# navigator8972/vae_assoc

Hardware: AMD Instinct MI355X
Metric: paired-samples/sec (img+jnt assoc-VAE train step) (higher is better)
Workload: dtype bf16

## Files before the change

vae_assoc_amd/csrc/avae_device.h:

```cpp
#pragma once
#include <hip/hip_runtime.h>
#include <stdint.h>

namespace avae {

constexpr int kMaxMod = 4;
constexpr int kThreads = 256;
constexpr int kTileBytesK = 128;
constexpr int kRowAlign = 256;
constexpr int kLatentRows = 16;
constexpr int kAdamRows = 16;
constexpr int kCostHist = 4096;

enum Kind : int {
    K_FWD_HIDDEN = 0,
    K_FWD_HEAD = 1,
    K_FWD_OUT_LOSS = 2,
    K_FWD_OUT_STORE = 3,
    K_DGRAD_HIDDEN = 4,
    K_DGRAD_LATENT = 5,
    K_WGRAD = 6,
    K_DGRAD_F32 = 10,
    K_LATENT = 7,
    K_COST = 8,
// ... 54 lines not shown
    int src_sb, src_sp;
    int ones;
    unsigned mg_ohw, mg_ow, mg_k, mg_cin;
};
constexpr int kMaxConvA = 12;
constexpr int kMaxItemsPerLaunch = 12;
constexpr int kMaxPf = 4;
struct LaunchArgs {
    int n_items;
    int grid_x;
    int sched;
    int n_pf;
    const void* pf_ptr[4];
    int pf_lines[4];
    const ConvA* conv_tab;
    WorkItem items[kMaxItemsPerLaunch];
};

struct TnItem {
    const void* A;
    const void* B;
    float* out;
    int M, N, K;
    int lda, ldb, ld0;
    int tiles_m, tiles_n;
    int ksplit, kchunk;
    int bias_row;
    int tile_off, tile_cnt;
    int conv;
    void* W; void* Wt;
    int ldw, ldt;
};
constexpr int kMaxTnItems = 32;
constexpr int kTnPieces = 8;
struct TnPiece { unsigned short item, tile_off, cum_end, pad; };
struct DevState;
struct TnLaunchArgs {
    int n_items;
    int grid_x;
    int xcd_group;
    int sched;
    int adam;
    long long d_theta, d_m, d_v;
    float beta1, beta2, eps;
    const DevState* st;
    const ConvA* conv_tab;
    int xcd_pieces;
    TnPiece pieces[8][kTnPieces];
    TnItem items[kMaxTnItems];
};
static_assert(sizeof(TnLaunchArgs) <= 4096, "kernel arguments are passed by value: 4 KiB");

struct DevState {
    long long step;
    float last_cost;
    float lr_t;
    float cost_hist[kCostHist];
};

struct AdamItem {
    float* theta;
    float* m;
    float* v;
    const float* g;
    void* W;
    void* Wt;
    int rows, cols;
    int ld, ldt;
    int tiles_r, tiles_c, tile_base;
    int ldw;
    void* Wadj; void* Wf;
    int ldadj, ldf, adj_k, adj_cin;
};

constexpr int kMaxAdamItems = 80;
struct AdamArgs {
    const AdamItem* items;
    int n_items;
    int base[kMaxAdamItems];
    int mode;
    int book;
// ... 219 lines not shown
```

vae_assoc_amd/csrc/avae_host.hip:

```cpp
#include "avae_device.h"
#include "../../include/avae.h"

#include <dlfcn.h>
#include <sched.h>
#include <unistd.h>

#include <algorithm>
#include <cmath>
#include <cstdio>
#include <cstdlib>
#include <cstring>
#include <functional>
#include <map>
#include <mutex>
#include <stdexcept>
#include <string>
#include <vector>

using namespace avae;

namespace {

thread_local std::string g_create_error;

// ... 168 lines not shown
    int bwd_split = 0;
    std::vector<Launch> wgrad_b[2];
    struct Range { size_t off, count; };
    std::vector<Range> ranges_b[2];
    int adam_first_b[2] = {0, 0}, adam_count_b[2] = {0, 0}, adam_blocks_b[2] = {0, 0};
    std::vector<AdamItem> adam_items_b;
    size_t off_adam_b = 0;
    void* comm = nullptr;
    int comm_world = 1, comm_rank = 0;
    bool comm_on = false;
    size_t off_wire = 0;
    unsigned char* ipc_block = nullptr;
    size_t ipc_bytes = 0;
    unsigned char* ipc_peer[kMaxWorld] = {nullptr, nullptr, nullptr, nullptr, nullptr, nullptr, nullptr, nullptr};
    bool ipc_opened[kMaxWorld] = {false, false, false, false, false, false, false, false};
    bool ipc_attached = false;
    IpcArgs ipc_args{};
    hipStream_t comm_stream = nullptr;
    hipEvent_t ev_grad[2] = {nullptr, nullptr}, ev_red[2] = {nullptr, nullptr};
    std::vector<StepGraph> g_dp[2];
    StepGraph g_dpm[2];
    bool dp_graph_failed = false;
    Launch cost_only;
    std::vector<AdamItem> adam_items;
    int adam_blocks = 0;
    struct Inf { std::vector<WorkItem> items; std::vector<Launch> launches; int rows = -1; size_t dev_off = 0; };
    std::vector<Inf> inf_enc, inf_dec;
    struct Serve { int bucket = 0; std::vector<WorkItem> items; std::vector<Launch> launches; hipGraphExec_t graph = nullptr; ServeArgs in;
                   Launch in_launch; bool fused_in = false;
                   ServeInArgs in_lean; int in_lean_grid = 0; bool lean_in = false; };
    std::vector<Serve> serve;
    size_t off_slot = 0;
    float* iw_buf = nullptr;
    size_t off_chain = 0;
    size_t off_consts = 0, off_conv_tab = 0;
    std::vector<ConvA> conv_tab;

    StepPlan plain, masked;
    unsigned char* pres_buf = nullptr;
    size_t pres_set = 0;

    hipStream_t last_stream = nullptr;
    bool has_last_stream = false;
    hipEvent_t ev_switch = nullptr;
    unsigned draw_id = 0;
    bool timing = false;
    bool debug_sync = false;
    std::vector<std::string> tnames;
    std::vector<TimingRec> trecs;

    template <typename T> T* at(size_t off) const { return reinterpret_cast<T*>(ws + off); }
    DevState* state() const { return at<DevState>(off_state); }
    float* grad() const { return at<float>(off_g); }
};

namespace {

inline int spread_ld(int ld, int KU, int es) {
    static const bool off = std::getenv("AVAE_NO_LD_SPREAD") != nullptr;
    return (!off && ((size_t)ld * es) % 512 == 0) ? ld + KU : ld;
}

Act make_act(Bump& b, int width, bool ones, int rows, int KU, int es, int ld = 0) {
    Act a;
    a.width = width;
    a.rows = rows;
// ... 751 lines not shown
            std::vector<std::vector<TnItem>> bins, bins2;
            if (!std::getenv("AVAE_TN_G") && G == 4 && n * 2 <= kMaxTnItems * 2) {
                const long r4 = pack(4, bins), r2 = pack(2, bins2);
                if (r2 < r4) { G = 2; bins.swap(bins2); }
            } else {
                pack(G, bins);
            }
            size_t groups = 0;
            for (const auto& bn : bins) groups = std::max(groups, bn.size());
            std::memset(L.targs.items, 0, sizeof(L.targs.items));
            for (size_t g = 0; g < groups; ++g)
                for (int p = 0; p < G; ++p) if (g < bins[p].size()) L.targs.items[g * G + p] = bins[p][g];
            n = (int)groups * G;
        }
        L.grid_x = SX;
        L.targs.n_items = n;
        L.targs.grid_x = L.grid_x;
        L.targs.xcd_group = G;
        L.grid_y = (n + G - 1) / G * G;
        L.blocks = L.grid_x * L.grid_y;
    } else {
        L.args.n_items = count;
        L.args.grid_x = L.grid_x;
        for (int i = 0; i < count; ++i) L.args.items[i] = items[first + i];
    }
    L.args.conv_tab = L.targs.conv_tab = h->at<ConvA>(h->off_conv_tab);
    if (const char* e = std::getenv("AVAE_SCHED")) L.args.sched = L.targs.sched = std::atoi(e);
    if (*next_slot > h->n_partial) throw Err("internal error: cost partial slots overflow");
    return L;
}

void dp_ranges(const avae_handle* h, int* n_buckets, std::vector<avae_handle::Range> (&out)[2]);

void xcd_pieces(Launch& L) {
    TnLaunchArgs& a = L.targs;
    std::vector<TnItem> layers;
    for (int i = 0; i < a.n_items; ++i) {
        const TnItem& e = a.items[i];
        if (e.tile_cnt <= 0) continue;
        bool seen = false;
        for (const TnItem& l : layers) seen = seen || l.out == e.out;
        if (seen) continue;
        TnItem l = e;
        l.tile_off = 0; l.tile_cnt = e.tiles_m * e.tiles_n;
        if (l.tile_cnt > 65535) return;
        layers.push_back(l);
    }
    long total = 0;
    for (const TnItem& l : layers) total += l.tile_cnt;
    if (layers.empty() || total > 8L * 65535) return;
    const int quota = (int)((total + 7) / 8);
    std::vector<int> order(layers.size());
    for (size_t i = 0; i < order.size(); ++i) order[i] = (int)i;
    std::stable_sort(order.begin(), order.end(), [&](int x, int y) { return layers[x].tile_cnt > layers[y].tile_cnt; });
    struct Bin { int load = 0; std::vector<TnPiece> pc; };
    Bin bins[8];
    for (int li : order) {
        int off = 0, left = layers[li].tile_cnt;
        while (left > 0) {
            int best = -1;
            for (int b = 0; b < 8; ++b)
                if ((int)bins[b].pc.size() < kTnPieces && bins[b].load + left <= quota && (best < 0 || bins[b].load > bins[best].load)) best = b;
            int take = left;
            if (best < 0) {
                for (int b = 0; b < 8; ++b)
                    if ((int)bins[b].pc.size() < kTnPieces && bins[b].load < quota && (best < 0 || bins[b].load < bins[best].load)) best = b;
                if (best < 0) return;
                take = std::min(left, quota - bins[best].load);
            }
            bins[best].load += take;
            bins[best].pc.push_back(TnPiece{(unsigned short)li, (unsigned short)off, (unsigned short)bins[best].load, 0});
            off += take; left -= take;
        }
    }
    int longest = 0;
    for (int b = 0; b < 8; ++b) {
        longest = std::max(longest, bins[b].load);
        for (int i = 0; i < kTnPieces; ++i)
            a.pieces[b][i] = i < (int)bins[b].pc.size() ? bins[b].pc[i] : TnPiece{0, 0, (unsigned short)bins[b].load, 0};
    }
    std::memset(a.items, 0, sizeof(a.items));
    for (size_t i = 0; i < layers.size(); ++i) a.items[i] = layers[i];
    a.n_items = (int)layers.size();
    a.xcd_pieces = 1;
    L.grid_x = 8 * longest; L.grid_y = 1; L.blocks = L.grid_x;
    a.grid_x = L.grid_x;
}

void build_training_plan(avae_handle* h) {
    h->items.clear(); h->plain.fwd.clear(); h->bwd.clear(); h->wgrad.clear(); h->conv_tab.clear();
    Builder bd(h, h->items, h->B, true);
    int slot = 0;
    int Lmax = 0;
    for (const Mod& md : h->mods) Lmax = std::max(Lmax, md.L);
    auto group = [&](const std::string& name, std::vector<Launch>& dst, auto&& fill) {
        const int first = (int)h->items.size();
        fill();
        const int count = (int)h->items.size() - first;
        if (count <= 0) return;
        dst.push_back(finish_launch(h, h->items, first, count, name, &slot));
    };
    auto fuse_tail = [&](std::vector<Launch>& ls, int mode) {
        if (ls.size() < 2 || std::getenv("AVAE_NO_TAIL")) return false;
        Launch& Lp = ls[ls.size() - 2];
        Launch& Lc = ls[ls.size() - 1];
        if (Lp.type != 0 || Lc.type != 0 || Lp.tn || Lc.tn || Lp.cfg != 3) return false;
        const int want_p = mode == 1 ? K_FWD_HEAD : K_DGRAD_LATENT, want_c = mode == 1 ? K_FWD_HIDDEN : K_DGRAD_HIDDEN;
        std::vector<int> prod(Lc.count, -1);
        for (int i = 0; i < Lc.count; ++i) {
            const WorkItem& c = h->items[Lc.first + i];
            if (c.kind != want_c || c.bias_ep || c.K > 2 * h->KU || c.N > 1024) return false;
            for (int k = 0; k < Lp.count; ++k) {
                const WorkItem& n = h->items[Lp.first + k];
                if (n.kind != want_p || n.M != c.M) continue;
                const void* res = mode == 1 ? n.out1 : n.out0;
                const int ldres = mode == 1 ? n.ld1 : n.ld0;
                if (res && res == c.A && ldres == c.lda) prod[i] = k;
            }
// ... 495 lines not shown
                g.block_base = base; base += (st.g.Cin * st.g.k * st.g.k * st.d.out + kThreads - 1) / kThreads;
            }
            L.blocks = base;
            if (base > 0) h->wgrad.push_back(L);
        }
    }
    h->wgrad_adam.clear();
    if (!any_conv && h->wgrad.size() == 1 && h->wgrad[0].tn && h->wgrad[0].cfg == 0 && h->wgrad[0].targs.xcd_group == 1
        && !std::getenv("AVAE_NO_LEAN") && !std::getenv("AVAE_NO_ADAM_FUSE")) {
        Launch L = h->wgrad[0];
        bool ok = true;
        for (int i = 0; i < L.targs.n_items && ok; ++i) {
            TnItem& t = L.targs.items[i];
            ok = t.ksplit <= 1 && t.bias_row == 0 && t.K > 0;
            const Dense* dm = nullptr;
            for (const Mod& md : h->mods) {
                auto look = [&](const Dense& d) { if (h->grad() + d.master == t.out) dm = &d; };
                for (const Dense& d : md.enc) look(d);
                look(md.head);
                for (const Dense& d : md.dec) look(d);
                look(md.outl);
            }
            ok = ok && dm && t.M == dm->in + 1 && t.N == dm->out && t.ld0 == dm->ld;
            if (ok) { t.W = h->at<void>(dm->W); t.Wt = h->at<void>(dm->Wt); t.ldw = dm->ldw; t.ldt = dm->ldt; }
        }
        if (ok) {
            L.cfg = 12; L.name = "wgrad+adam";
            L.targs.adam = 1;
            L.targs.d_theta = h->at<float>(h->off_theta) - h->grad();
            L.targs.d_m = h->at<float>(h->off_m) - h->grad();
            L.targs.d_v = h->at<float>(h->off_v) - h->grad();
            L.targs.beta1 = h->cfg.beta1; L.targs.beta2 = h->cfg.beta2; L.targs.eps = h->cfg.adam_eps;
            L.targs.st = h->state();
            if (!std::getenv("AVAE_NO_XCD_PIECES")) xcd_pieces(L);
            h->wgrad_adam.push_back(L);
        }
    }
    if (!std::getenv("AVAE_NO_WARM")) {
        std::vector<Launch*> seq;
        for (Launch& L : h->plain.fwd) seq.push_back(&L);
        for (Launch& L : h->bwd) seq.push_back(&L);
        for (size_t i = 0; i < seq.size(); ++i) {
            Launch& L = *seq[i];
            if (L.type != 0 || L.tn || (L.cfg != 2 && L.cfg != 6)) continue;
            for (size_t j = i + 1; j < seq.size(); ++j) {
                const Launch& Nx = *seq[j];
                if (Nx.type != 0) continue;
                if (Nx.tn) break;
                for (int k = 0; k < Nx.args.n_items && L.args.n_pf < kMaxPf; ++k) {
                    const WorkItem& w = Nx.args.items[k];
                    if (!is_gemm(w.kind) || w.kind == K_WGRAD) continue;
                    const long bytes = (long)w.N * w.ldb * h->es;
                    if (bytes < 128 * 1024) continue;
                    L.args.pf_ptr[L.args.n_pf] = w.B; L.args.pf_lines[L.args.n_pf] = (int)(bytes / 128); ++L.args.n_pf;
                }
                break;
            }
        }
    }
    {
        const int first = (int)h->items.size();
        h->items.push_back(bd.cost(false));
        h->cost_only = finish_launch(h, h->items, first, 1, "cost_reduce", &slot);
    }

    h->adam_items.clear();
    int base = 0;
// ... 116 lines not shown
    avae_handle* h; hipStream_t s; bool on; hipEvent_t a = nullptr, b = nullptr; int id = 0;
    Timed(avae_handle* h_, hipStream_t s_, const std::string& name) : h(h_), s(s_), on(h_->timing && h_->trecs.size() < 200000) {
        if (!on) return;
        id = tname_id(h, name);
        HIP_OK(hipEventCreate(&a)); HIP_OK(hipEventCreate(&b));
        t_launch_events = LaunchEvents{a, b};
    }
    ~Timed() {
        if (!on) return;
        if (t_launch_events.start) {
            t_launch_events = LaunchEvents{nullptr, nullptr};
            (void)hipEventRecord(a, s); (void)hipEventRecord(b, s);
        }
        h->trecs.push_back(TimingRec{a, b, id});
    }
};

Launch relocated(const avae_handle* h, const Launch& L0, int j) {
    Launch L = L0;
    const unsigned char* lo = h->ws + h->stage_lo;
    const unsigned char* hi = lo + h->stage_bytes;
    const size_t delta = (size_t)j * h->stage_bytes;
    auto fix = [&](auto& ptr) {
        const unsigned char* q = reinterpret_cast<const unsigned char*>(ptr);
        if (q >= lo && q < hi) ptr = reinterpret_cast<std::remove_reference_t<decltype(ptr)>>(const_cast<unsigned char*>(q) + delta);
    };
    for (int i = 0; i < L.args.n_items && L.type == 0; ++i) {
        WorkItem& w = L.args.items[i];
        fix(w.A); fix(w.B); fix(w.out0); fix(w.out1); fix(w.out2); fix(w.aux0); fix(w.aux1); fix(w.aux2); fix(w.eps);
        fix(w.tail_w); fix(w.tail_out); fix(w.tail_aux);
        if (w.present) w.present += (size_t)j * h->pres_set;
    }
    for (int i = 0; i < L.targs.n_items && L.type == 0; ++i) { TnItem& t = L.targs.items[i]; fix(t.A); fix(t.B); fix(t.out); }
    for (int i = 0; i < L.ga.n_seg && L.type == 1; ++i) fix(L.ga.seg[i].src);
    return L;
}

void run_launch(avae_handle* h, const Launch& L, hipStream_t s, unsigned long long* stamps, int stamp) {
    Timed t(h, s, L.name);
    if (L.type == 1) launch_gather(h->cfg.compute_dtype, L.ga, L.blocks, s);
    else if (L.type == 2) launch_col2im(h->cfg.compute_dtype, L.ca, L.blocks, s);
    else if (L.type == 3) launch_reduce(L.ra, L.blocks, s);
    else if (L.type == 4) launch_thin(h->cfg.compute_dtype, L.ta, L.blocks, s);
    else if (L.type == 5) launch_colsum(L.ra, L.blocks, s);
    else if (L.type == 6) launch_wadj(h->cfg.compute_dtype, L.wa, L.blocks, s);
    else if (L.type == 7) launch_gperm(L.gp, L.blocks, s);
    else if (L.type == 8) launch_rowsum(h->cfg.compute_dtype, L.rs, L.blocks, s);
    else if (L.type == 9) launch_sums(L.ra, L.blocks, s);
    else if (L.cfg == 13) launch_chain2(h->cfg.compute_dtype, L.args, L.grid_x, L.grid_y, L.lds, h->at<unsigned>(h->off_chain), h->at<unsigned>(h->off_chain) + kMaxMod * 64, s);
    else if (L.cfg == 11) launch_small_head(h->cfg.compute_dtype, L.lean_act, L.args, L.grid_x, L.grid_y, L.lds, s, stamps, stamp);
    else if (L.cfg == 10) launch_small_latb(h->cfg.compute_dtype, L.lean_act, L.args, L.grid_x, L.grid_y, L.lds, h->state(), s, stamps, stamp);
    else if (L.cfg == 9) launch_small_loss(h->cfg.compute_dtype, L.args, L.grid_x, L.grid_y, L.lds, s, stamps, stamp);
    else if (L.cfg == 7) launch_small(h->cfg.compute_dtype, L.args, L.grid_x, L.grid_y, L.lds, s, stamps, stamp);
    else if (L.tn && L.cfg == 12) launch_small_tn(h->cfg.compute_dtype, L.targs, L.grid_x, L.grid_y, s, stamps, stamp);
    else if (L.tn) launch_grouped_tn(h->cfg.compute_dtype, L.cfg, L.targs, L.grid_x, L.grid_y, L.lds, h->state(), s, stamps, stamp);
    else launch_grouped(h->cfg.compute_dtype, L.cfg, L.args, L.grid_x, L.grid_y, L.lds, h->state(), s, stamps, stamp);
    LAUNCH_OK(L.name);
    if (h->debug_sync) {
        std::fprintf(stderr, "[avae] launch %s type=%d cfg=%d items=%d blocks=%d\n", L.name.c_str(), L.type, L.cfg, L.count, L.blocks);
        for (int i = 0; i < L.args.n_items && L.type == 0; ++i)
            std::fprintf(stderr, "        item kind=%d M=%d N=%d K=%d lda=%d ldb=%d tiles=%dx%d\n", L.args.items[i].kind, L.args.items[i].M,
                         L.args.items[i].N, L.args.items[i].K, L.args.items[i].lda, L.args.items[i].ldb, L.args.items[i].tiles_m, L.args.items[i].tiles_n);
        for (int i = 0; i < L.ga.n_seg && L.type == 1; ++i)
            std::fprintf(stderr, "        gather B=%d IH=%d Cin=%d OH=%d k=%d so=%d d=%d pad=%d sb=%d sp=%d ones=%d ldp=%d tiles=%dx%d\n", L.ga.seg[i].g.B, L.ga.seg[i].g.IH,
                         L.ga.seg[i].g.Cin, L.ga.seg[i].g.OH, L.ga.seg[i].g.k, L.ga.seg[i].g.so, L.ga.seg[i].g.d, L.ga.seg[i].g.pad, L.ga.seg[i].g.src_sb, L.ga.seg[i].g.src_sp,
                         L.ga.seg[i].g.ones, L.ga.seg[i].ldp, L.ga.seg[i].tiles_r, L.ga.seg[i].tiles_c);
// ... 111 lines not shown
            size_t n_root = 0;
            HIP_OK(hipGraphGetRootNodes(sg.graph, nullptr, &n_root));
            if (n_root != 1) throw Err("internal error: the captured step is not a chain");
            HIP_OK(hipGraphGetRootNodes(sg.graph, &sg.prep, &n_root));
            hipGraphNodeType ty;
            HIP_OK(hipGraphNodeGetType(sg.prep, &ty));
            if (ty != hipGraphNodeTypeKernel) throw Err("internal error: the captured step does not start with the staging kernel");
        }
        HIP_OK(hipGraphInstantiate(&sg.exec, sg.graph, nullptr, nullptr, 0));
        if (!with_prep) { HIP_OK(hipGraphDestroy(sg.graph)); sg.graph = nullptr; }
    } catch (...) { sg.release(); throw; }
    return sg;
}

void patch_prep(avae_handle* h, const StepGraph& sg, const float* const* x, const int32_t* x_ld, const float* eps,
                int n_steps = 1, const uint8_t* present = nullptr) {
    PrepArgs a = make_prep_batch(h, x, x_ld, eps, h->B, 0x7261696eull, n_steps, present);
    void* kp[1] = {&a};
    hipKernelNodeParams np;
    std::memset(&np, 0, sizeof(np));
    np.func = const_cast<void*>(prep_kernel(h->cfg.compute_dtype, present != nullptr));
    np.gridDim = dim3((a.total_tiles + a.eps_blocks) * n_steps); np.blockDim = dim3(kThreads);
    np.sharedMemBytes = 0; np.kernelParams = kp; np.extra = nullptr;
    HIP_OK(hipGraphExecKernelNodeSetParams(sg.exec, sg.prep, &np));
}

void fill_ones(avae_handle* h, const Act& a, hipStream_t s) {
    if (!a.ones) return;
    const unsigned bits = h->es == 2 ? 0x3F80u : 0x3F800000u;
    launch_fill(h->at<void>(a.rm), h->es, bits, a.width, a.ld, h->B, s);
    LAUNCH_OK("fill");
}

void step_body(avae_handle* h, const std::vector<Launch>& fwd, hipStream_t s, int j, int stamp_base = -1) {
    auto sb = [&](size_t k) { return stamp_base < 0 ? -1 : stamp_base + (int)k; };
    run_set(h, fwd, 0, fwd.size(), j, s, stamp_base);
    run_set(h, h->bwd, 0, h->bwd.size(), j, s, sb(fwd.size()));
    if (!h->wgrad_adam.empty()) {
        run_set(h, h->wgrad_adam, 0, h->wgrad_adam.size(), j, s, sb(fwd.size() + h->bwd.size()));
        return;
    }
    run_set(h, h->wgrad, 0, h->wgrad.size(), j, s, sb(fwd.size() + h->bwd.size()));
    run_adam(h, 0, s);
}

void capture_plan(avae_handle* h, StepPlan& p, const uint8_t* present) {
    std::vector<const float*> x0(h->M, h->at<float>(h->mods[0].X32));
    try {
        p.full = capture(h, [&](hipStream_t cs) {
            run_prep_batch(h, x0.data(), nullptr, nullptr, h->B, 0x7261696eull, cs, present);
            step_body(h, p.fwd, cs, 0, 0);
        }, true);
        for (int gi = 0; gi < 2; ++gi) p.multi[gi] = capture(h, [&](hipStream_t cs) {
            run_prep_batch(h, x0.data(), nullptr, nullptr, h->B, 0x7261696eull, cs, present, kMultiSizes[gi]);
            for (int j = 0; j < kMultiSizes[gi]; ++j) step_body(h, p.fwd, cs, j);
        }, true);
        p.eval = capture(h, [&](hipStream_t cs) { run_launches(h, p.fwd, cs); run_launch(h, h->cost_only, cs, nullptr, -1); });
    } catch (...) { p.release(); throw; }
}

void init_device(avae_handle* h) {
    hipStream_t s = h->cap_stream;
    HIP_OK(hipMemsetAsync(h->ws, 0, h->ws_bytes, s));
    for (const Mod& md : h->mods) {
        for (int j = 0; j < kMultiSteps; ++j) {
            Act x = md.X0;
            x.rm += (size_t)j * h->stage_bytes;
            fill_ones(h, x, s);
        }
        for (const Act& a : md.E) fill_ones(h, a, s);
        fill_ones(h, md.Z, s);
        for (const Act& a : md.D) fill_ones(h, a, s);
        if (md.conv && md.cdec[3].dense_map) fill_ones(h, md.cdec[3].Y, s);
    }
    build_training_plan(h);
    HIP_OK(hipMemcpyAsync(h->at<void>(h->off_adam), h->adam_items.data(), h->adam_items.size() * sizeof(AdamItem), hipMemcpyHostToDevice, s));
    HIP_OK(hipMemcpyAsync(h->at<void>(h->off_adam_b), h->adam_items_b.data(), h->adam_items_b.size() * sizeof(AdamItem), hipMemcpyHostToDevice, s));
    {
        static const unsigned char c32_bf16[32] = {0, 0, 0, 0, 0, 0, 0, 0, 0, 0, 0, 0, 0, 0, 0, 0, 0x80, 0x3F};
        static const unsigned char c32_f32[32] = {0, 0, 0, 0, 0, 0, 0, 0, 0, 0, 0, 0, 0, 0, 0, 0, 0, 0, 0x80, 0x3F};
        HIP_OK(hipMemcpyAsync(h->at<void>(h->off_consts), h->es == 2 ? c32_bf16 : c32_f32, 32, hipMemcpyHostToDevice, s));
        if (!h->conv_tab.empty()) {
            const unsigned char* lo = h->ws + h->stage_lo;
            for (const ConvA& c : h->conv_tab)
                if (reinterpret_cast<const unsigned char*>(c.src) >= lo && reinterpret_cast<const unsigned char*>(c.src) < lo + h->stage_bytes * kMultiSteps)
                    throw Err("internal error: an implicit patch matrix on a staged input (not relocatable per step)");
            HIP_OK(hipMemcpyAsync(h->at<void>(h->off_conv_tab), h->conv_tab.data(), h->conv_tab.size() * sizeof(ConvA), hipMemcpyHostToDevice, s));
        }
// ... 528 lines not shown
            b.at(i);
            run_prep_batch(h, b.x, x_ld, b.eps, h->B, 0x7261696eull, s, nullptr, n);
            for (int j = 0; j < n; ++j) dp_step(h, j, s);
        }
    } else {
        if (!h->timing) i = replay_runs(h, p.multi, b, n_steps, s, [&](int gi) { return p.multi[gi].exec != nullptr; });
        for (; i < n_steps; ++i) {
            b.at(i);
            train_one(h, p, b.x, x_ld, b.pres, b.eps, s);
        }
    }
    fetch_cost(h, cost_host, true, s);
}

void eval_cost(avae_handle* h, StepPlan& p, const float* const* x_dev, const int32_t* x_ld, const uint8_t* present, const float* eps_dev,
               float* cost_host, hipStream_t s) {
    run_prep_batch(h, x_dev, x_ld, eps_dev, h->B, 0x6576616cull  | (unsigned long long)next_draw(h, eps_dev) << 34, s, present);
    if (p.eval.exec && !h->timing) HIP_OK(hipGraphLaunch(p.eval.exec, s));
    else { run_launches(h, p.fwd, s); run_launch(h, h->cost_only, s, nullptr, -1); }
    fetch_cost(h, cost_host, false, s);
}

void destroy_handle(avae_handle* h) {
    int prev_dev = -1;
    if (hipGetDevice(&prev_dev) != hipSuccess) prev_dev = -1;
    (void)hipSetDevice(h->cfg.device);
    (void)hipDeviceSynchronize();
    h->plain.release();
    h->masked.release();
    for (StepGraph& g : h->g_dpm) g.release();
    for (std::vector<StepGraph>& v : h->g_dp) for (StepGraph& g : v) g.release();
    for (avae_handle::Serve& sv : h->serve) if (sv.graph) (void)hipGraphExecDestroy(sv.graph);
    if (h->iw_buf) (void)hipFree(h->iw_buf);
    if (h->pres_buf) (void)hipFree(h->pres_buf);
    if (h->ev_switch) (void)hipEventDestroy(h->ev_switch);
    if (h->comm) { try { (void)Rccl::get().destroy(h->comm); } catch (...) {} }
    for (int r = 0; r < kMaxWorld; ++r) if (h->ipc_opened[r] && h->ipc_peer[r]) (void)hipIpcCloseMemHandle(h->ipc_peer[r]);
    if (h->ipc_block) (void)hipFree(h->ipc_block);
    for (int b = 0; b < 2; ++b) { if (h->ev_grad[b]) (void)hipEventDestroy(h->ev_grad[b]); if (h->ev_red[b]) (void)hipEventDestroy(h->ev_red[b]); }
    if (h->comm_stream) (void)hipStreamDestroy(h->comm_stream);
    for (TimingRec& r : h->trecs) { (void)hipEventDestroy(r.a); (void)hipEventDestroy(r.b); }
    if (h->cap_stream) (void)hipStreamDestroy(h->cap_stream);
    if (h->own_ws && h->ws) (void)hipFree(h->ws);
    if (prev_dev >= 0 && prev_dev != h->cfg.device) (void)hipSetDevice(prev_dev);
    delete h;
}

}

extern "C" {

int avae_workspace_bytes(const avae_config* cfg, size_t* bytes) {
    try {
        if (!cfg || !bytes) throw Err("null argument");
        check_config(*cfg);
        avae_handle tmp;
        tmp.cfg = *cfg;
        plan_memory(&tmp);
        *bytes = tmp.ws_bytes;
        return 0;
    } catch (const std::exception& e) { g_create_error = e.what(); return 2; }
}

int avae_create(const avae_config* cfg, avae_handle** out) {
    avae_handle* h = nullptr;
    try {
// ... 677 lines not shown
```

vae_assoc_amd/csrc/avae_kernels.hip:

```cpp
#include "avae_device.h"
#include <hip/hip_ext.h>
#include <stdexcept>
#include "../../include/avae.h"

namespace avae {

typedef __attribute__((ext_vector_type(8))) __bf16 bf16x8;
typedef __attribute__((ext_vector_type(4))) __bf16 bf16x4;
typedef __attribute__((ext_vector_type(4))) float f32x4;
typedef __attribute__((ext_vector_type(4))) unsigned u32x4;


template <typename CT> __device__ __forceinline__ CT to_ct(float v);
template <> __device__ __forceinline__ float to_ct<float>(float v) { return v; }
template <> __device__ __forceinline__ __bf16 to_ct<__bf16>(float v) { return (__bf16)v; }

__device__ __forceinline__ float bf16_bits_to_float(unsigned b) { return __uint_as_float(b << 16); }

template <typename CT> __device__ __forceinline__ void load4(const CT* p, float v[4]);
template <> __device__ __forceinline__ void load4<float>(const float* p, float v[4]) {
    float4 t = *reinterpret_cast<const float4*>(p);
    v[0] = t.x; v[1] = t.y; v[2] = t.z; v[3] = t.w;
}
template <> __device__ __forceinline__ void load4<__bf16>(const __bf16* p, float v[4]) {
// ... 1664 lines not shown
#define K_LATB_B(A) k_small_latb<__bf16, A>
#define K_LATB_F(A) k_small_latb<float, A>
    if (compute_dtype == AVAE_BF16) {
        switch (act) {
            case AVAE_ACT_RELU: AVAE_LAUNCH((K_LATB_B(AVAE_ACT_RELU)), grid, block, lds_bytes, s, args, st, stamps, launch_id); break;
            case AVAE_ACT_SOFTPLUS: AVAE_LAUNCH((K_LATB_B(AVAE_ACT_SOFTPLUS)), grid, block, lds_bytes, s, args, st, stamps, launch_id); break;
            case AVAE_ACT_SIGMOID: AVAE_LAUNCH((K_LATB_B(AVAE_ACT_SIGMOID)), grid, block, lds_bytes, s, args, st, stamps, launch_id); break;
            case AVAE_ACT_TANH: AVAE_LAUNCH((K_LATB_B(AVAE_ACT_TANH)), grid, block, lds_bytes, s, args, st, stamps, launch_id); break;
            default: AVAE_LAUNCH((K_LATB_B(AVAE_ACT_IDENTITY)), grid, block, lds_bytes, s, args, st, stamps, launch_id); break;
        }
    } else {
        switch (act) {
            case AVAE_ACT_RELU: AVAE_LAUNCH((K_LATB_F(AVAE_ACT_RELU)), grid, block, lds_bytes, s, args, st, stamps, launch_id); break;
            case AVAE_ACT_SOFTPLUS: AVAE_LAUNCH((K_LATB_F(AVAE_ACT_SOFTPLUS)), grid, block, lds_bytes, s, args, st, stamps, launch_id); break;
            case AVAE_ACT_SIGMOID: AVAE_LAUNCH((K_LATB_F(AVAE_ACT_SIGMOID)), grid, block, lds_bytes, s, args, st, stamps, launch_id); break;
            case AVAE_ACT_TANH: AVAE_LAUNCH((K_LATB_F(AVAE_ACT_TANH)), grid, block, lds_bytes, s, args, st, stamps, launch_id); break;
            default: AVAE_LAUNCH((K_LATB_F(AVAE_ACT_IDENTITY)), grid, block, lds_bytes, s, args, st, stamps, launch_id); break;
        }
    }
#undef K_LATB_B
#undef K_LATB_F
}

template <typename CT, bool ADAM>
__global__ void __launch_bounds__(kThreads) k_small_tn(const TnLaunchArgs args, unsigned long long* stamps, int launch_id) {
    constexpr int BM = 64, RING = 4, ES = (int)sizeof(CT), EPR = kTileBytesK / ES, NCH = 4;
    constexpr int kStage = 2 * BM * kTileBytesK;
    unsigned char* smem = avae_dyn_smem;
#ifdef AVAE_STAMPS
    unsigned long long sv[kStampWords] = {0, 0, 0, 0, 0, 0, 0, 0};
#endif
    AVAE_STAMP(0)
    const int part = blockIdx.x & 7, idx = blockIdx.x >> 3;
    int entry = blockIdx.y, t_piece = -1;
    if (args.xcd_pieces) {
        const TnPiece* row = args.pieces[part];
        int e = 0, lo = 0;
#pragma unroll
        for (int i = 0; i < kTnPieces; ++i) { const int ce = row[i].cum_end; if (idx >= ce) { e = i + 1; lo = ce; } }
        if (e >= kTnPieces) return;
        entry = row[e].item; t_piece = row[e].tile_off + idx - lo;
    }
    const TnItem w = args.items[entry];
    asm volatile("" :: "s"(w.A), "s"(w.B), "s"(w.out), "s"(w.lda), "s"(w.ldb), "s"(w.K), "s"(w.ld0), "s"(w.tile_off));
    float lr_t = 0.f;
    if constexpr (ADAM) lr_t = args.st->lr_t;
    int t;
    if (t_piece >= 0) {
        t = t_piece;
    } else {
        const int nt = w.tile_cnt;
        const int q = nt >> 3, r = nt & 7;
        if (idx >= q + (part < r ? 1 : 0)) return;
        t = (part < r ? part * (q + 1) : r * (q + 1) + (part - r) * q) + idx + w.tile_off;
    }
    const int tid = threadIdx.x, lane = tid & 63, wave = __builtin_amdgcn_readfirstlane(tid >> 6);
    const int wr = wave >> 1, wc = wave & 1, fr = lane & 15, fq = lane >> 4;
    const int tm = t / w.tiles_n, tn = t - tm * w.tiles_n;
    const int m0 = tm * BM, n0 = tn * BM;
    const int nk = (w.K * ES) / kTileBytesK;
    typedef const __attribute__((address_space(1))) void* gp_t;
    typedef __attribute__((address_space(3))) void* lp_t;
    const unsigned char* src[NCH];
    size_t kadv[NCH];
#pragma unroll
    for (int c = 0; c < NCH; ++c) {
        const int r = (c * 4 + wave) * 8 + (lane >> 3);
        const bool is_a = c < 2;
        const int rr = is_a ? r : r - BM, sub = rr / EPR, k = rr - sub * EPR;
        const int lc = (lane & 7) ^ tn_swz<CT>(k);
        const size_t ld_b = (size_t)(is_a ? w.lda : w.ldb) * ES;
        kadv[c] = (size_t)EPR * ld_b;
        src[c] = reinterpret_cast<const unsigned char*>(is_a ? w.A : w.B) + (size_t)(is_a ? m0 : n0) * ES + (size_t)k * ld_b + (size_t)sub * kTileBytesK + lc * 16;
    }
#define AVAE_T_DMA(kt, buf)                                                                                             \
    { _Pragma("unroll") for (int c = 0; c < NCH; ++c)                                                                   \
        __builtin_amdgcn_global_load_lds((gp_t)(src[c] + (size_t)(kt) * kadv[c]), (lp_t)(smem + (buf) * kStage + (c * 4 + wave) * 1024), 16, 0, 0); }
    int offA[2], offB[2];
#pragma unroll
    for (int i = 0; i < 2; ++i) { offA[i] = tn_frag_off<CT>(wr * 32 + i * 16, lane); offB[i] = BM * kTileBytesK + tn_frag_off<CT>(wc * 32 + i * 16, lane); }
    AVAE_STAMP(1)
    const int npro = nk < RING - 1 ? nk : RING - 1;
    for (int p = 0; p < npro; ++p) AVAE_T_DMA(p, p)
    const int c4 = (tid & 15) * 4;
    f32x4 pth[4], pmm[4], pvv[4];
    auto fetch_state = [&]() {
#pragma unroll
        for (int k = 0; k < 4; ++k) {
            const int grow = m0 + (tid >> 4) + 16 * k, gcol = n0 + c4;
            const bool ok = grow < w.M && gcol < w.N;
            const float* gp = w.out + (size_t)(ok ? grow : m0) * w.ld0 + (ok ? gcol : n0);
            pth[k] = *reinterpret_cast<const f32x4*>(gp + args.d_theta);
// ... 44 lines not shown
                const int col = n0 + wc * 32 + j * 16 + 4 * fq;
                if (row < w.M && col < w.N) {
                    const float g[4] = {acc[i][j][0], acc[i][j][1], acc[i][j][2], acc[i][j][3]};
                    store_row<float>(w.out + (size_t)row * w.ld0 + col, g, w.N - col);
                }
            }
        }
    } else {
        constexpr int LDT = 65;
        float* T = reinterpret_cast<float*>(smem);
        fetch_state();
        lds_barrier();
#pragma unroll
        for (int i = 0; i < 2; ++i)
#pragma unroll
            for (int j = 0; j < 2; ++j)
#pragma unroll
                for (int e = 0; e < 4; ++e) T[(wr * 32 + i * 16 + fr) * LDT + wc * 32 + j * 16 + 4 * fq + e] = acc[i][j][e];
        lds_barrier();
        const float omb1 = 1.0f - args.beta1, omb2 = 1.0f - args.beta2;
        const int r4 = (tid & 15) * 4;
        float g[4][4], th[4][4], m[4][4], v[4][4];
#pragma unroll
        for (int k = 0; k < 4; ++k) {
            const int r = (tid >> 4) + 16 * k;
#pragma unroll
            for (int e = 0; e < 4; ++e) { g[k][e] = T[r * LDT + c4 + e]; th[k][e] = pth[k][e]; m[k][e] = pmm[k][e]; v[k][e] = pvv[k][e]; }
#pragma unroll
            for (int e = 0; e < 4; ++e) adam_update(g[k][e], m[k][e], v[k][e], th[k][e], omb1, omb2, lr_t, args.eps);
#pragma unroll
            for (int e = 0; e < 4; ++e) T[r * LDT + c4 + e] = th[k][e];
        }
        const bool full = m0 + BM <= w.M && n0 + BM <= w.N;
        auto store_group = [&](int k, float* gp, CT* wp) {
            store4<float>(gp, g[k]);
            store4<float>(gp + args.d_theta, th[k]); store4<float>(gp + args.d_m, m[k]); store4<float>(gp + args.d_v, v[k]);
            store4<CT>(wp, th[k]);
        };
        if (full) {
#pragma unroll
            for (int k = 0; k < 4; ++k) {
                const int grow = m0 + (tid >> 4) + 16 * k, gcol = n0 + c4;
                store_group(k, w.out + (size_t)grow * w.ld0 + gcol, reinterpret_cast<CT*>(w.W) + (size_t)grow * w.ldw + gcol);
            }
        } else {
#pragma unroll
            for (int k = 0; k < 4; ++k) {
                const int grow = m0 + (tid >> 4) + 16 * k, gcol = n0 + c4;
                float* gp = w.out + (size_t)grow * w.ld0 + gcol;
                CT* wp = reinterpret_cast<CT*>(w.W) + (size_t)grow * w.ldw + gcol;
                const int nv = w.N - gcol;
                if (grow < w.M && nv >= 4) {
                    store_group(k, gp, wp);
                } else if (grow < w.M && nv > 0) {
#pragma unroll
                    for (int e = 0; e < 3; ++e) if (e < nv) {
                        gp[e] = g[k][e]; gp[args.d_theta + e] = th[k][e]; gp[args.d_m + e] = m[k][e]; gp[args.d_v + e] = v[k][e]; wp[e] = to_ct<CT>(th[k][e]);
                    }
                    asm volatile("; partial quad" ::: "memory");
                }
            }
        }
        lds_barrier();
#pragma unroll
        for (int k = 0; k < 4; ++k) {
            const int c = (tid >> 4) + 16 * k;
            const int gcol = n0 + c, grow = m0 + r4;
            float t[4];
#pragma unroll
            for (int e = 0; e < 4; ++e) t[e] = T[(r4 + e) * LDT + c];
            CT* tp = reinterpret_cast<CT*>(w.Wt) + (size_t)gcol * w.ldt + grow;
            if (full) store4<CT>(tp, t);
            else if (gcol < w.N && grow < w.M) store_row<CT>(tp, t, w.M - grow);
        }
    }
    AVAE_STAMP(4)
    AVAE_STAMP_FLUSH()
}
void launch_small_tn(int compute_dtype, const TnLaunchArgs& args, int grid_x, int grid_y, hipStream_t s, unsigned long long* stamps, int launch_id) {
    const dim3 grid(grid_x, grid_y), block(kThreads);
    const int lds_bytes = 4 * 2 * 64 * kTileBytesK;
    if (compute_dtype == AVAE_BF16) {
        if (args.adam) AVAE_LAUNCH((k_small_tn<__bf16, true>), grid, block, lds_bytes, s, args, stamps, launch_id);
        else AVAE_LAUNCH((k_small_tn<__bf16, false>), grid, block, lds_bytes, s, args, stamps, launch_id);
    } else {
        if (args.adam) AVAE_LAUNCH((k_small_tn<float, true>), grid, block, lds_bytes, s, args, stamps, launch_id);
        else AVAE_LAUNCH((k_small_tn<float, false>), grid, block, lds_bytes, s, args, stamps, launch_id);
    }
}

// ... 1410 lines not shown
```

Before: 4.778 million.

## Schedule weight-gradient tiles per XCD via device block table; skip intermediate gradient stores

Replaces the per-XCD piece list in kernel arguments with a device-resident table of per-block descriptors. Tiles are balanced across the eight XCDs by element count rather than tile count and sorted largest-first within each bin. Separately, fused wgrad+Adam launches skip writing the raw fp32 gradient on every step of a multi-step graph except the last, cutting global store traffic. This costs an extra descriptor load per block and a device allocation, and makes the stored gradient stale on intermediate steps.

New measurement: 4.826 million, median of 6. +1.0%, better.

```diff
diff --git a/vae_assoc_amd/csrc/avae_device.h b/vae_assoc_amd/csrc/avae_device.h
--- a/vae_assoc_amd/csrc/avae_device.h
+++ b/vae_assoc_amd/csrc/avae_device.h
@@ -110,8 +110,17 @@
     int ldw, ldt;
 };
 constexpr int kMaxTnItems = 32;
-constexpr int kTnPieces = 8;
-struct TnPiece { unsigned short item, tile_off, cum_end, pad; };
+struct TnBlock {
+    const void* A; const void* B;
+    float* out;
+    void* W; void* Wt;
+    int M, N, K, lda, ldb, ld0, ldw, ldt;
+    int m0, n0;
+    int flags;
+    int pad[3];
+};
+constexpr int kTnRelocA = 1, kTnRelocB = 2, kTnEmpty = 4;
+static_assert(sizeof(TnBlock) == 96, "TnBlock: 96 bytes, two scalar loads from one base");
 struct DevState;
 struct TnLaunchArgs {
     int n_items;
@@ -124,7 +133,9 @@
     const DevState* st;
     const ConvA* conv_tab;
     int xcd_pieces;
-    TnPiece pieces[8][kTnPieces];
+    int no_g;
+    long long reloc;
+    const TnBlock* blk;
     TnItem items[kMaxTnItems];
 };
 static_assert(sizeof(TnLaunchArgs) <= 4096, "kernel arguments are passed by value: 4 KiB");
diff --git a/vae_assoc_amd/csrc/avae_host.hip b/vae_assoc_amd/csrc/avae_host.hip
--- a/vae_assoc_amd/csrc/avae_host.hip
+++ b/vae_assoc_amd/csrc/avae_host.hip
@@ -224,6 +224,7 @@
     std::vector<Serve> serve;
     size_t off_slot = 0;
     float* iw_buf = nullptr;
+    TnBlock* tn_blk = nullptr;
     size_t off_chain = 0;
     size_t off_consts = 0, off_conv_tab = 0;
     std::vector<ConvA> conv_tab;
@@ -1041,7 +1042,7 @@
 
 void dp_ranges(const avae_handle* h, int* n_buckets, std::vector<avae_handle::Range> (&out)[2]);
 
-void xcd_pieces(Launch& L) {
+void xcd_pieces(avae_handle* h, Launch& L) {
     TnLaunchArgs& a = L.targs;
     std::vector<TnItem> layers;
     for (int i = 0; i < a.n_items; ++i) {
@@ -1052,47 +1053,80 @@
         if (seen) continue;
         TnItem l = e;
         l.tile_off = 0; l.tile_cnt = e.tiles_m * e.tiles_n;
-        if (l.tile_cnt > 65535) return;
         layers.push_back(l);
     }
-    long total = 0;
-    for (const TnItem& l : layers) total += l.tile_cnt;
-    if (layers.empty() || total > 8L * 65535) return;
-    const int quota = (int)((total + 7) / 8);
+    long tiles = 0, total = 0;
+    for (const TnItem& l : layers) { tiles += l.tile_cnt; total += (long)l.M * l.N; }
+    if (layers.empty() || tiles > 8L * 65535) return;
+    const int BM = 64;
+    auto elems = [&](const TnItem& l, int t) {
+        const int tm = t / l.tiles_n, tn = t - tm * l.tiles_n;
+        return (long)std::min(BM, l.M - tm * BM) * std::min(BM, l.N - tn * BM);
+    };
+    const long quota = (total + 7) / 8;
+    const size_t cap = std::max<size_t>((tiles + 7) / 8, 64);
     std::vector<int> order(layers.size());
     for (size_t i = 0; i < order.size(); ++i) order[i] = (int)i;
-    std::stable_sort(order.begin(), order.end(), [&](int x, int y) { return layers[x].tile_cnt > layers[y].tile_cnt; });
-    struct Bin { int load = 0; std::vector<TnPiece> pc; };
+    std::stable_sort(order.begin(), order.end(), [&](int x, int y) { return (long)layers[x].M * layers[x].N > (long)layers[y].M * layers[y].N; });
+    struct Tile { int layer, t; long e; };
+    struct Bin { long load = 0; std::vector<Tile> ts; };
     Bin bins[8];
     for (int li : order) {
-        int off = 0, left = layers[li].tile_cnt;
-        while (left > 0) {
+        const TnItem& l = layers[li];
+        int off = 0;
+        long left = (long)l.M * l.N;
+        while (off < l.tile_cnt) {
             int best = -1;
             for (int b = 0; b < 8; ++b)
-                if ((int)bins[b].pc.size() < kTnPieces && bins[b].load + left <= quota && (best < 0 || bins[b].load > bins[best].load)) best = b;
-            int take = left;
+                if (bins[b].ts.size() + (size_t)(l.tile_cnt - off) <= cap && bins[b].load + left <= quota
+                    && (best < 0 || bins[b].load > bins[best].load)) best = b;
+            int end = l.tile_cnt;
             if (best < 0) {
                 for (int b = 0; b < 8; ++b)
-                    if ((int)bins[b].pc.size() < kTnPieces && bins[b].load < quota && (best < 0 || bins[b].load < bins[best].load)) best = b;
-                if (best < 0) return;
-                take = std::min(left, quota - bins[best].load);
-            }
-            bins[best].load += take;
-            bins[best].pc.push_back(TnPiece{(unsigned short)li, (unsigned short)off, (unsigned short)bins[best].load, 0});
-            off += take; left -= take;
-        }
-    }
-    int longest = 0;
-    for (int b = 0; b < 8; ++b) {
-        longest = std::max(longest, bins[b].load);
-        for (int i = 0; i < kTnPieces; ++i)
-            a.pieces[b][i] = i < (int)bins[b].pc.size() ? bins[b].pc[i] : TnPiece{0, 0, (unsigned short)bins[b].load, 0};
-    }
+                    if (bins[b].ts.size() < cap && (best < 0 || bins[b].load < bins[best].load)) best = b;
+                if (best < 0) throw Err("internal error: weight-gradient tiles beyond the XCDs' capacity");
+                const size_t room = cap - bins[best].ts.size();
+                long load = bins[best].load + elems(l, off);
+                for (end = off + 1; end < l.tile_cnt && (size_t)(end - off) < room && load + elems(l, end) <= quota; ++end) load += elems(l, end);
+            }
+            for (; off < end; ++off) {
+                const long e = elems(l, off);
+                bins[best].ts.push_back(Tile{li, off, e});
+                bins[best].load += e; left -= e;
+            }
+        }
+    }
+    size_t longest = 0;
+    for (Bin& b : bins) {
+        std::stable_sort(b.ts.begin(), b.ts.end(), [](const Tile& x, const Tile& y) { return x.e > y.e; });
+        longest = std::max(longest, b.ts.size());
+    }
+    const unsigned char* lo = h->ws + h->stage_lo;
+    const unsigned char* hi = lo + h->stage_bytes;
+    auto staged = [&](const void* p) { const unsigned char* q = reinterpret_cast<const unsigned char*>(p); return q >= lo && q < hi; };
+    std::vector<TnBlock> blk(8 * longest);
+    for (size_t x = 0; x < blk.size(); ++x) {
+        TnBlock& d = blk[x];
+        std::memset(&d, 0, sizeof(d));
+        const Bin& b = bins[x % 8];
+        if (x / 8 >= b.ts.size()) { d.flags = kTnEmpty; continue; }
+        const Tile& tl = b.ts[x / 8];
+        const TnItem& l = layers[tl.layer];
+        const int tm = tl.t / l.tiles_n, tn = tl.t - tm * l.tiles_n;
+        d.A = l.A; d.B = l.B; d.out = l.out; d.W = l.W; d.Wt = l.Wt;
+        d.M = l.M; d.N = l.N; d.K = l.K; d.lda = l.lda; d.ldb = l.ldb; d.ld0 = l.ld0; d.ldw = l.ldw; d.ldt = l.ldt;
+        d.m0 = tm * BM; d.n0 = tn * BM;
+        d.flags = (staged(l.A) ? kTnRelocA : 0) | (staged(l.B) ? kTnRelocB : 0);
+    }
+    if (h->tn_blk) { HIP_OK(hipFree(h->tn_blk)); h->tn_blk = nullptr; }
+    HIP_OK(hipMalloc(&h->tn_blk, blk.size() * sizeof(TnBlock)));
+    HIP_OK(hipMemcpy(h->tn_blk, blk.data(), blk.size() * sizeof(TnBlock), hipMemcpyHostToDevice));
     std::memset(a.items, 0, sizeof(a.items));
     for (size_t i = 0; i < layers.size(); ++i) a.items[i] = layers[i];
     a.n_items = (int)layers.size();
     a.xcd_pieces = 1;
-    L.grid_x = 8 * longest; L.grid_y = 1; L.blocks = L.grid_x;
+    a.blk = h->tn_blk;
+    L.grid_x = (int)blk.size(); L.grid_y = 1; L.blocks = L.grid_x;
     a.grid_x = L.grid_x;
 }
 
@@ -1654,7 +1688,7 @@
             L.targs.d_v = h->at<float>(h->off_v) - h->grad();
             L.targs.beta1 = h->cfg.beta1; L.targs.beta2 = h->cfg.beta2; L.targs.eps = h->cfg.adam_eps;
             L.targs.st = h->state();
-            if (!std::getenv("AVAE_NO_XCD_PIECES")) xcd_pieces(L);
+            if (!std::getenv("AVAE_NO_XCD_PIECES")) xcd_pieces(h, L);
             h->wgrad_adam.push_back(L);
         }
     }
@@ -1837,6 +1871,7 @@
         if (w.present) w.present += (size_t)j * h->pres_set;
     }
     for (int i = 0; i < L.targs.n_items && L.type == 0; ++i) { TnItem& t = L.targs.items[i]; fix(t.A); fix(t.B); fix(t.out); }
+    L.targs.reloc = (long long)delta;
     for (int i = 0; i < L.ga.n_seg && L.type == 1; ++i) fix(L.ga.seg[i].src);
     return L;
 }
@@ -2014,12 +2049,14 @@
     LAUNCH_OK("fill");
 }
 
-void step_body(avae_handle* h, const std::vector<Launch>& fwd, hipStream_t s, int j, int stamp_base = -1) {
+void step_body(avae_handle* h, const std::vector<Launch>& fwd, hipStream_t s, int j, int stamp_base = -1, bool store_g = true) {
     auto sb = [&](size_t k) { return stamp_base < 0 ? -1 : stamp_base + (int)k; };
     run_set(h, fwd, 0, fwd.size(), j, s, stamp_base);
     run_set(h, h->bwd, 0, h->bwd.size(), j, s, sb(fwd.size()));
     if (!h->wgrad_adam.empty()) {
-        run_set(h, h->wgrad_adam, 0, h->wgrad_adam.size(), j, s, sb(fwd.size() + h->bwd.size()));
+        std::vector<Launch> wa = h->wgrad_adam;
+        for (Launch& L : wa) L.targs.no_g = store_g ? 0 : 1;
+        run_set(h, wa, 0, wa.size(), j, s, sb(fwd.size() + h->bwd.size()));
         return;
     }
     run_set(h, h->wgrad, 0, h->wgrad.size(), j, s, sb(fwd.size() + h->bwd.size()));
@@ -2035,7 +2072,7 @@
         }, true);
         for (int gi = 0; gi < 2; ++gi) p.multi[gi] = capture(h, [&](hipStream_t cs) {
             run_prep_batch(h, x0.data(), nullptr, nullptr, h->B, 0x7261696eull, cs, present, kMultiSizes[gi]);
-            for (int j = 0; j < kMultiSizes[gi]; ++j) step_body(h, p.fwd, cs, j);
+            for (int j = 0; j < kMultiSizes[gi]; ++j) step_body(h, p.fwd, cs, j, -1, j + 1 == kMultiSizes[gi]);
         }, true);
         p.eval = capture(h, [&](hipStream_t cs) { run_launches(h, p.fwd, cs); run_launch(h, h->cost_only, cs, nullptr, -1); });
     } catch (...) { p.release(); throw; }
@@ -2630,6 +2667,7 @@
     for (std::vector<StepGraph>& v : h->g_dp) for (StepGraph& g : v) g.release();
     for (avae_handle::Serve& sv : h->serve) if (sv.graph) (void)hipGraphExecDestroy(sv.graph);
     if (h->iw_buf) (void)hipFree(h->iw_buf);
+    if (h->tn_blk) (void)hipFree(h->tn_blk);
     if (h->pres_buf) (void)hipFree(h->pres_buf);
     if (h->ev_switch) (void)hipEventDestroy(h->ev_switch);
     if (h->comm) { try { (void)Rccl::get().destroy(h->comm); } catch (...) {} }
diff --git a/vae_assoc_amd/csrc/avae_kernels.hip b/vae_assoc_amd/csrc/avae_kernels.hip
--- a/vae_assoc_amd/csrc/avae_kernels.hip
+++ b/vae_assoc_amd/csrc/avae_kernels.hip
@@ -1720,32 +1720,36 @@
 #endif
     AVAE_STAMP(0)
     const int part = blockIdx.x & 7, idx = blockIdx.x >> 3;
-    int entry = blockIdx.y, t_piece = -1;
-    if (args.xcd_pieces) {
-        const TnPiece* row = args.pieces[part];
-        int e = 0, lo = 0;
-#pragma unroll
-        for (int i = 0; i < kTnPieces; ++i) { const int ce = row[i].cum_end; if (idx >= ce) { e = i + 1; lo = ce; } }
-        if (e >= kTnPieces) return;
-        entry = row[e].item; t_piece = row[e].tile_off + idx - lo;
-    }
-    const TnItem w = args.items[entry];
-    asm volatile("" :: "s"(w.A), "s"(w.B), "s"(w.out), "s"(w.lda), "s"(w.ldb), "s"(w.K), "s"(w.ld0), "s"(w.tile_off));
+    TnItem w;
+    int m0, n0;
     float lr_t = 0.f;
-    if constexpr (ADAM) lr_t = args.st->lr_t;
-    int t;
-    if (t_piece >= 0) {
-        t = t_piece;
+    const DevState* st = args.st;
+    if (args.blk) {
+        const TnBlock d = args.blk[blockIdx.x];
+        if constexpr (ADAM) lr_t = st->lr_t;
+        const long long reloc = args.reloc;
+        asm volatile("" :: "s"(d.A), "s"(d.B), "s"(d.out), "s"(d.W), "s"(d.Wt), "s"(d.M), "s"(d.N), "s"(d.K), "s"(d.lda), "s"(d.ldb),
+                     "s"(d.ld0), "s"(d.ldw), "s"(d.ldt), "s"(d.m0), "s"(d.n0), "s"(d.flags), "s"(lr_t), "s"(reloc));
+        if (d.flags & kTnEmpty) return;
+        w.A = reinterpret_cast<const unsigned char*>(d.A) + ((d.flags & kTnRelocA) ? reloc : 0);
+        w.B = reinterpret_cast<const unsigned char*>(d.B) + ((d.flags & kTnRelocB) ? reloc : 0);
+        w.out = d.out; w.W = d.W; w.Wt = d.Wt;
+        w.M = d.M; w.N = d.N; w.K = d.K; w.lda = d.lda; w.ldb = d.ldb; w.ld0 = d.ld0; w.ldw = d.ldw; w.ldt = d.ldt;
+        m0 = d.m0; n0 = d.n0;
     } else {
+        const int entry = blockIdx.y;
+        w = args.items[entry];
+        asm volatile("" :: "s"(w.A), "s"(w.B), "s"(w.out), "s"(w.lda), "s"(w.ldb), "s"(w.K), "s"(w.ld0), "s"(w.tile_off));
+        if constexpr (ADAM) lr_t = st->lr_t;
         const int nt = w.tile_cnt;
         const int q = nt >> 3, r = nt & 7;
         if (idx >= q + (part < r ? 1 : 0)) return;
-        t = (part < r ? part * (q + 1) : r * (q + 1) + (part - r) * q) + idx + w.tile_off;
+        const int t = (part < r ? part * (q + 1) : r * (q + 1) + (part - r) * q) + idx + w.tile_off;
+        const int tm = t / w.tiles_n, tn = t - tm * w.tiles_n;
+        m0 = tm * BM; n0 = tn * BM;
     }
     const int tid = threadIdx.x, lane = tid & 63, wave = __builtin_amdgcn_readfirstlane(tid >> 6);
     const int wr = wave >> 1, wc = wave & 1, fr = lane & 15, fq = lane >> 4;
-    const int tm = t / w.tiles_n, tn = t - tm * w.tiles_n;
-    const int m0 = tm * BM, n0 = tn * BM;
     const int nk = (w.K * ES) / kTileBytesK;
     typedef const __attribute__((address_space(1))) void* gp_t;
     typedef __attribute__((address_space(3))) void* lp_t;
@@ -1856,8 +1860,9 @@
             for (int e = 0; e < 4; ++e) T[r * LDT + c4 + e] = th[k][e];
         }
         const bool full = m0 + BM <= w.M && n0 + BM <= w.N;
+        const bool store_g = !args.no_g;
         auto store_group = [&](int k, float* gp, CT* wp) {
-            store4<float>(gp, g[k]);
+            if (store_g) store4<float>(gp, g[k]);
             store4<float>(gp + args.d_theta, th[k]); store4<float>(gp + args.d_m, m[k]); store4<float>(gp + args.d_v, v[k]);
             store4<CT>(wp, th[k]);
         };
@@ -1879,7 +1884,8 @@
                 } else if (grow < w.M && nv > 0) {
 #pragma unroll
                     for (int e = 0; e < 3; ++e) if (e < nv) {
-                        gp[e] = g[k][e]; gp[args.d_theta + e] = th[k][e]; gp[args.d_m + e] = m[k][e]; gp[args.d_v + e] = v[k][e]; wp[e] = to_ct<CT>(th[k][e]);
+                        if (store_g) gp[e] = g[k][e];
+                        gp[args.d_theta + e] = th[k][e]; gp[args.d_m + e] = m[k][e]; gp[args.d_v + e] = v[k][e]; wp[e] = to_ct<CT>(th[k][e]);
                     }
                     asm volatile("; partial quad" ::: "memory");
                 }
```
